# fudan-zvg/PARTNER

Measured on AMD Instinct MI355X. Metric: frames/sec polar voxelize+PFN+BEV+head, 30k-pt sweep (whole job), higher is better.
Workload: dtype f32

## Files before the change

partner_amd/csrc/pillar_rows.hip:

```cpp
#include "pn_common.h"
#include "wino_planes.h"
#include <algorithm>

namespace {

using f32x4 = __attribute__((ext_vector_type(4))) float;

#ifndef PN_ROWS_EXP
#define PN_ROWS_EXP 0
#endif
constexpr int RW_LD = 132;
constexpr int RW_MAXLIST = 256;

struct RowsArgs {
  const float* canvas;
  const uint32_t* keys;
  const int32_t* row_start;
  const float* w;
  const float* scale;
  const float* shift;
  float* planes;
  float* out;
  int B, T, R, OH, OW, Wq, in_ps, in_co, act, cout, cout_pad, out_ps, out_co, v_cap;
  unsigned plane_floats, canvas_bytes, w_bytes;
};

template <int NS>
__global__ __launch_bounds__(512) void pillar_rows_kernel(RowsArgs a) {
  extern __shared__ __attribute__((aligned(16))) float smem[];
  float* tile = smem;
  int* lists = reinterpret_cast<int*>(smem + (size_t)a.OW * RW_LD);
  int* cnt = lists + 3 * 2 * RW_MAXLIST;
  const int tid = threadIdx.x, lane = tid & 63, wv = __builtin_amdgcn_readfirstlane(tid >> 6);
  const int go = blockIdx.x;
  const int b = go / a.OH, oy = go - b * a.OH;

  int run_lo = 0, run_hi = 0;
  if (wv < 3) {
    const int iy = 2 * oy - 1 + wv;
    if (iy >= 0 && iy < a.T) {
      run_lo = a.row_start[b * a.T + iy];
      run_hi = a.row_start[b * a.T + iy + 1];
    }
  }
  {
    const f32x4 z = {0.f, 0.f, 0.f, 0.f};
    f32x4* t4 = reinterpret_cast<f32x4*>(tile);
    for (int i = tid; i < a.OW * RW_LD / 4; i += 512) t4[i] = z;
  }
  if (wv < 3) {
    const int iy = 2 * oy - 1 + wv;
    int ne = 0, no = 0;
    if (iy >= 0 && iy < a.T) {
      const int gi = b * a.T + iy;
      const int lo = min(run_lo, a.v_cap), hi = min(run_hi, a.v_cap);
      const uint32_t key0 = (uint32_t)gi * (uint32_t)a.R;
      int* le = lists + (wv * 2 + 0) * RW_MAXLIST;
      int* lo_ = lists + (wv * 2 + 1) * RW_MAXLIST;
      for (int base = lo; base < hi; base += 64) {
        const int i = base + lane;
        const bool live = i < hi;
        const int ix = live ? (int)(a.keys[i] - key0) : 0;
        const bool odd = live && (ix & 1), even = live && !(ix & 1);
        const unsigned long long me = __ballot(even), mo = __ballot(odd);
        const unsigned long long below = (1ull << lane) - 1ull;
        if (even) le[ne + __popcll(me & below)] = ix;
        if (odd) lo_[no + __popcll(mo & below)] = ix;
        ne += __popcll(me);
        no += __popcll(mo);
      }
    }
    if (lane == 0) {
      cnt[wv * 2] = ne;
      cnt[wv * 2 + 1] = no;
    }
  }
  __syncthreads();

  const __amdgpu_buffer_rsrc_t rsrc_c = __builtin_amdgcn_make_buffer_rsrc(const_cast<float*>(a.canvas), 0, a.canvas_bytes, 0x00020000);
  const __amdgpu_buffer_rsrc_t rsrc_w = __builtin_amdgcn_make_buffer_rsrc(const_cast<float*>(a.w), 0, a.w_bytes, 0x00020000);
  const int j = lane & 15, kq = lane >> 4;
  const int c0 = wv * 16;
  const bool cols_live = c0 < a.cout;
  const unsigned w_lane = (unsigned)(((c0 + j) * 4 + kq) * 16);
  const unsigned w_slab = (unsigned)a.cout_pad * 64u;
  auto load_w = [&](int tap, f32x4 (&f)[NS]) __attribute__((always_inline)) {
#pragma unroll
    for (int s = 0; s < NS; ++s)
      f[s] = __builtin_bit_cast(f32x4, __builtin_amdgcn_raw_buffer_load_b128(rsrc_w, (cols_live && !(PN_ROWS_EXP & 4)) ? w_lane : 0xffffffffu, (unsigned)(tap * NS + s) * w_slab, 0));
  };
  auto add_to_tile = [&](int ox, const f32x4 acc) __attribute__((always_inline)) {
    f32x4* p = reinterpret_cast<f32x4*>(tile + (size_t)ox * RW_LD + c0 + 4 * kq);
    *p = *p + acc;
  };
  f32x4 w0[NS], w1[NS], w2[NS];
  auto row_live = [&](int kh) { const int iy = 2 * oy - 1 + kh; return iy >= 0 && iy < a.T && !(PN_ROWS_EXP & 1); };
  if (row_live(0)) load_w(1, w1);
  else load_w(3 + 1, w1);
#pragma unroll
  for (int kh = 0; kh < 3; ++kh) {
    if (!row_live(kh)) continue;
    const int iy = 2 * oy - 1 + kh;
    const unsigned row_pix = (unsigned)(b * a.T + iy) * (unsigned)a.R;
    const int ne = cnt[kh * 2], no = cnt[kh * 2 + 1];
    const int te = (ne + 15) >> 4, nu = te + ((no + 15) >> 4);
    const int* le = lists + (kh * 2 + 0) * RW_MAXLIST;
    const int* lo_ = lists + (kh * 2 + 1) * RW_MAXLIST;
    auto unit_ix = [&](int u) {
      const bool odd = u >= te;
      const int idx = (odd ? u - te : u) * 16 + j;
      return idx < (odd ? no : ne) ? (odd ? lo_[idx] : le[idx]) : -1;
    };
    auto request = [&](int ix, f32x4 (&xf)[NS]) __attribute__((always_inline)) {
      const unsigned voff = (ix >= 0 && !(PN_ROWS_EXP & 4)) ? ((row_pix + (unsigned)ix) * (unsigned)a.in_ps + (unsigned)a.in_co + 4u * (unsigned)kq) * 4u : 0xffffffffu;
#pragma unroll
      for (int s2 = 0; s2 < NS; ++s2) xf[s2] = __builtin_bit_cast(f32x4, __builtin_amdgcn_raw_buffer_load_b128(rsrc_c, voff, (unsigned)s2 * 64u, 0));
    };
    auto unit = [&](int u, int ix, const f32x4 (&xf)[NS], int ix_next, f32x4 (&xn)[NS]) __attribute__((always_inline)) {
      if (u + 1 < nu) request(ix_next, xn);
      f32x4 p = {0.f, 0.f, 0.f, 0.f}, q = {0.f, 0.f, 0.f, 0.f};
      if (u < te) {
#pragma unroll
        for (int s2 = 0; s2 < ((PN_ROWS_EXP & 8) ? 0 : NS); s2 += 2)
#pragma unroll
          for (int m = 0; m < 4; ++m) {
            p = __builtin_amdgcn_mfma_f32_16x16x4f32(w1[s2][m], xf[s2][m], p, 0, 0, 0);
            q = __builtin_amdgcn_mfma_f32_16x16x4f32(w1[s2 + 1][m], xf[s2 + 1][m], q, 0, 0, 0);
          }
        if (ix >= 0) add_to_tile(ix >> 1, p + q);
        if (u + 1 == te && kh < 2) load_w((kh + 1) * 3 + 1, w1);
      } else {
#pragma unroll
        for (int s2 = 0; s2 < ((PN_ROWS_EXP & 8) ? 0 : NS); ++s2)
#pragma unroll
          for (int m = 0; m < 4; ++m) {
            p = __builtin_amdgcn_mfma_f32_16x16x4f32(w0[s2][m], xf[s2][m], p, 0, 0, 0);
            q = __builtin_amdgcn_mfma_f32_16x16x4f32(w2[s2][m], xf[s2][m], q, 0, 0, 0);
          }
        if (ix >= 0 && ((ix + 1) >> 1) < a.OW) add_to_tile((ix + 1) >> 1, p);
        if (ix >= 0) add_to_tile((ix - 1) >> 1, q);
      }
    };
    f32x4 xa[NS], xb[NS];
    int ixa = nu > 0 ? unit_ix(0) : -1, ixb = -1;
    if (nu > 0) request(ixa, xa);
    if (no > 0) {
      load_w(kh * 3 + 0, w0);
      load_w(kh * 3 + 2, w2);
    }
    if (te == 0 && kh < 2) load_w((kh + 1) * 3 + 1, w1);
#pragma unroll 1
    for (int u = 0; u < nu; u += 2) {
      ixb = u + 1 < nu ? unit_ix(u + 1) : -1;
      unit(u, ixa, xa, ixb, xb);
      if (u + 1 < nu) {
        ixa = u + 2 < nu ? unit_ix(u + 2) : -1;
        unit(u + 1, ixb, xb, ixa, xa);
      }
    }
  }
  __syncthreads();

  const f32x4 z = {0.f, 0.f, 0.f, 0.f};
  const int c4n = a.cout >> 2;
  if (PN_ROWS_EXP & 2) return;
  if (a.planes) {
    for (int it = tid; it < c4n * a.Wq; it += 512) {
      const int c4 = it / a.Wq, xq = it - c4 * a.Wq;
      f32x4 sc = {1.f, 1.f, 1.f, 1.f}, sh = z;
      if (a.scale) sc = *reinterpret_cast<const f32x4*>(a.scale + c4 * 4);
      if (a.shift) sh = *reinterpret_cast<const f32x4*>(a.shift + c4 * 4);
      f32x4 d[6];
#pragma unroll
      for (int i = 0; i < 6; ++i) {
        const int ox = 4 * xq - 1 + i;
        if (ox < 0 || ox >= a.OW) {
          d[i] = z;
        } else {
          const f32x4 s = *reinterpret_cast<const f32x4*>(tile + (size_t)ox * RW_LD + c4 * 4);
#pragma unroll
          for (int c = 0; c < 4; ++c) d[i][c] = pn::apply_act(fmaf(s[c], sc[c], sh[c]), a.act);
        }
      }
      f32x4 vv[6];
      pn::wino4_input_transform4(d, vv);
      pn::wino4_store_planes(a.planes, vv, c4, c4n, a.plane_floats, b, oy, xq, a.OH, a.Wq);
    }
  }
  if (a.out) {
    float* orow = a.out + ((size_t)go * a.OW) * a.out_ps + a.out_co;
    for (int it = tid; it < a.OW * c4n; it += 512) {
      const int ox = it / c4n, c4 = it - ox * c4n;
      f32x4 sc = {1.f, 1.f, 1.f, 1.f}, sh = z;
      if (a.scale) sc = *reinterpret_cast<const f32x4*>(a.scale + c4 * 4);
      if (a.shift) sh = *reinterpret_cast<const f32x4*>(a.shift + c4 * 4);
      const f32x4 s = *reinterpret_cast<const f32x4*>(tile + (size_t)ox * RW_LD + c4 * 4);
      f32x4 y;
#pragma unroll
      for (int c = 0; c < 4; ++c) y[c] = pn::apply_act(fmaf(s[c], sc[c], sh[c]), a.act);
      *reinterpret_cast<f32x4*>(orow + (size_t)ox * a.out_ps + c4 * 4) = y;
    }
  }
}

__global__ void pack_pillar_rows_weight_kernel(const float* __restrict__ w, int cout, int cin, int cout_pad, float* __restrict__ packed, size_t total) {
  for (size_t i = blockIdx.x * (size_t)blockDim.x + threadIdx.x; i < total; i += (size_t)gridDim.x * blockDim.x) {
    const int m = (int)(i & 3), kq = (int)((i >> 2) & 3);
    size_t r = i >> 4;
    const int co = (int)(r % cout_pad);
    r /= cout_pad;
    const int ns = cin / 16;
    const int s = (int)(r % ns), tap = (int)(r / ns);
    const int ci = 16 * s + 4 * kq + m;
    packed[i] = co < cout ? w[((size_t)co * cin + ci) * 9 + tap] : 0.f;
  }
}

static int rows_cout_pad(int cout) { return pn::cdiv(cout, 16) * 16; }

}

extern "C" {

int pn_pillar_conv_rows_supported(int batch, int h, int w, int cin, int cout, int stride) {
  if (stride != 2 || batch < 1 || h < 2 || w < 8 || (w & 7) || w > 2 * RW_MAXLIST) return 0;
  const int ow = (w - 1) / 2 + 1, wq = ow / 4;
  if (ow % 4 || !(wq == 16 || wq == 32 || wq == 64)) return 0;
  if (!(cin == 32 || cin == 64 || cin == 128) || cout < 4 || cout > 128 || (cout & 3)) return 0;
  return 1;
}

size_t pn_pillar_conv_rows_packed_weight_floats(int cout, int cin) { return (size_t)9 * cin * rows_cout_pad(cout); }

int pn_pack_pillar_conv_rows_weight_f32(const float* w_oihw, int cout, int cin, float* packed, pn_stream_t stream) {
  PN_REQUIRE(w_oihw && packed && cout >= 1 && cin >= 16 && cin % 16 == 0, "pack_pillar_conv_rows_weight: bad arguments");
  const size_t total = pn_pillar_conv_rows_packed_weight_floats(cout, cin);
  hipLaunchKernelGGL(pack_pillar_rows_weight_kernel, dim3((unsigned)std::min<size_t>(2048, (total + 255) / 256)), dim3(256), 0, pn::S(stream), w_oihw, cout, cin,
                     rows_cout_pad(cout), packed, total);
  return pn::check_launch("pack_pillar_rows_weight_kernel");
}

int pn_pillar_conv3x3_rows_f32(const float* canvas, int batch, int h, int w, int cin, int in_pixel_stride, int in_channel_offset, const uint32_t* unq_keys,
                               const int32_t* row_start, int v_capacity, const float* packed_rows_w, int cout, const float* scale, const float* shift, int act,
                               float* planes, float* out, int out_pixel_stride, int out_channel_offset, pn_stream_t stream) {
  PN_REQUIRE(canvas && unq_keys && row_start && packed_rows_w && (planes || out), "pillar_conv_rows: null pointer");
  PN_REQUIRE(pn_pillar_conv_rows_supported(batch, h, w, cin, cout, 2), "pillar_conv_rows: shape not covered (see pn_pillar_conv_rows_supported)");
  PN_REQUIRE(in_pixel_stride % 4 == 0 && in_channel_offset % 4 == 0 && in_channel_offset + cin <= in_pixel_stride && ((uintptr_t)canvas & 15) == 0,
             "pillar_conv_rows: the canvas slice must be 16-byte aligned");
  PN_REQUIRE(!out || (out_pixel_stride % 4 == 0 && out_channel_offset % 4 == 0 && out_channel_offset + cout <= out_pixel_stride && ((uintptr_t)out & 15) == 0),
             "pillar_conv_rows: the output slice must be 16-byte aligned");
  PN_REQUIRE(((uintptr_t)scale & 15) == 0 && ((uintptr_t)shift & 15) == 0 && ((uintptr_t)planes & 15) == 0, "pillar_conv_rows: 16-byte aligned tables");
  const unsigned long long cb = (unsigned long long)batch * h * w * in_pixel_stride * 4ull;
  PN_REQUIRE(cb < (1ull << 32), "pillar_conv_rows: canvases of 4 GiB or more are not addressable by the buffer descriptor");
  RowsArgs a{};
  a.canvas = canvas; a.keys = unq_keys; a.row_start = row_start; a.w = packed_rows_w; a.scale = scale; a.shift = shift; a.planes = planes; a.out = out;
  a.B = batch; a.T = h; a.R = w; a.OH = (h - 1) / 2 + 1; a.OW = (w - 1) / 2 + 1; a.Wq = a.OW / 4;
  a.in_ps = in_pixel_stride; a.in_co = in_channel_offset; a.act = act; a.cout = cout; a.cout_pad = rows_cout_pad(cout);
  a.out_ps = out_pixel_stride; a.out_co = out_channel_offset; a.v_cap = v_capacity;
  a.plane_floats = (unsigned)((size_t)batch * (a.OH + 2) * a.Wq * 4);
  a.canvas_bytes = (unsigned)cb;
  a.w_bytes = (unsigned)(pn_pillar_conv_rows_packed_weight_floats(cout, cin) * 4);
  const size_t smem = ((size_t)a.OW * RW_LD + 3 * 2 * RW_MAXLIST + 8) * sizeof(float);
  pn::ProfileSlot slot;
  const bool prof = pn::take_profile_slot(slot);
  hipStream_t st = pn::S(stream);
  const dim3 grid((unsigned)(batch * a.OH));
#define PN_ROWS_LAUNCH(NS)                                                                                                                  \
  do {                                                                                                                                      \
    static bool done[64] = {false};                                                                                                         \
    if (pn::first_use_on_device(done))                                                                                                      \
      (void)hipFuncSetAttribute(reinterpret_cast<const void*>(&pillar_rows_kernel<NS>), hipFuncAttributeMaxDynamicSharedMemorySize, 160 * 1024); \
    if (prof) hipExtLaunchKernelGGL(pillar_rows_kernel<NS>, grid, dim3(512), smem, st, slot.start, slot.stop, 0, a);                         \
    else hipLaunchKernelGGL(pillar_rows_kernel<NS>, grid, dim3(512), smem, st, a);                                                          \
  } while (0)
  if (cin == 128) PN_ROWS_LAUNCH(8);
  else if (cin == 64) PN_ROWS_LAUNCH(4);
  else PN_ROWS_LAUNCH(2);
#undef PN_ROWS_LAUNCH
  return pn::check_launch("pillar_rows_kernel");
}

}
```

Measured before the change: 1834.

## Split pillar-row conv blocks by output-channel band and column segment

Restructures the sparse pillar-row convolution kernel so each block handles one output-channel band (NW waves of 16 channels) and optionally a column segment with a halo, in place of a 512-thread block covering all channels of a row. This gives a larger grid with smaller LDS footprints, adds an XCD-aware block-index swizzle, and replaces the two-buffer unit ping-pong with separate even/odd loops that issue next-unit canvas loads interleaved between MFMA groups under sched_barriers. The aim is more occupancy and better latency hiding, at the cost of each block re-scanning the row's key lists and re-loading weights for its band. An env var can force the geometry, and the default picks 4-wave channel bands when OW is at least 128.

Result: no change. 1847 (median of 6 runs) (+0.7%).

```diff
diff --git a/partner_amd/csrc/pillar_rows.hip b/partner_amd/csrc/pillar_rows.hip
--- a/partner_amd/csrc/pillar_rows.hip
+++ b/partner_amd/csrc/pillar_rows.hip
@@ -1,6 +1,7 @@
 #include "pn_common.h"
 #include "wino_planes.h"
 #include <algorithm>
+#include <cstdlib>
 
 namespace {
 
@@ -9,8 +10,15 @@
 #ifndef PN_ROWS_EXP
 #define PN_ROWS_EXP 0
 #endif
-constexpr int RW_LD = 132;
 constexpr int RW_MAXLIST = 256;
+
+template <int CS, int NW>
+struct RowsGeom {
+  static constexpr int HALO = CS > 1 ? 1 : 0;
+  static constexpr int LD = 16 * NW + 4;
+  static constexpr int LCAP = RW_MAXLIST / CS + 2 * HALO;
+  static size_t smem_bytes(int ow) { return ((size_t)(ow / CS + 2 * HALO) * LD + 3 * 2 * LCAP + 8) * sizeof(float); }
+};
 
 struct RowsArgs {
   const float* canvas;
@@ -21,19 +29,28 @@
   const float* shift;
   float* planes;
   float* out;
-  int B, T, R, OH, OW, Wq, in_ps, in_co, act, cout, cout_pad, out_ps, out_co, v_cap;
+  int B, T, R, OH, OW, Wq, in_ps, in_co, act, cout, cout_pad, out_ps, out_co, v_cap, ncb;
   unsigned plane_floats, canvas_bytes, w_bytes;
 };
 
-template <int NS>
-__global__ __launch_bounds__(512) void pillar_rows_kernel(RowsArgs a) {
+template <int NS, int CS, int NW>
+__global__ __launch_bounds__(64 * NW) __attribute__((amdgpu_waves_per_eu(NW == 4 ? 3 : 2))) void pillar_rows_kernel(RowsArgs a) {
+  using G = RowsGeom<CS, NW>;
+  constexpr int HALO = G::HALO, LD = G::LD, LCAP = G::LCAP, NT = 64 * NW;
   extern __shared__ __attribute__((aligned(16))) float smem[];
+  const int OWS = a.OW / CS, TP = OWS + 2 * HALO;
   float* tile = smem;
-  int* lists = reinterpret_cast<int*>(smem + (size_t)a.OW * RW_LD);
-  int* cnt = lists + 3 * 2 * RW_MAXLIST;
+  int* lists = reinterpret_cast<int*>(smem + (size_t)TP * LD);
+  int* cnt = lists + 3 * 2 * LCAP;
   const int tid = threadIdx.x, lane = tid & 63, wv = __builtin_amdgcn_readfirstlane(tid >> 6);
-  const int go = blockIdx.x;
+  int bid = blockIdx.x;
+  if (!(PN_ROWS_EXP & 16) && !(gridDim.x & 7)) bid = (bid & 7) * (int)(gridDim.x >> 3) + (bid >> 3);
+  const int go = bid / (CS * a.ncb), band = bid - go * (CS * a.ncb);
+  const int seg = band / a.ncb, cb = band - seg * a.ncb;
   const int b = go / a.OH, oy = go - b * a.OH;
+  const int x0 = seg * OWS, x1 = x0 + OWS;
+  const int tx0 = max(x0 - HALO, 0), tx1 = min(x1 + HALO, a.OW);
+  const int ix_lo = CS > 1 ? 2 * x0 - 3 : 0, ix_hi = CS > 1 ? 2 * x1 + 1 : a.R;
 
   int run_lo = 0, run_hi = 0;
   if (wv < 3) {
@@ -46,7 +63,7 @@
   {
     const f32x4 z = {0.f, 0.f, 0.f, 0.f};
     f32x4* t4 = reinterpret_cast<f32x4*>(tile);
-    for (int i = tid; i < a.OW * RW_LD / 4; i += 512) t4[i] = z;
+    for (int i = tid; i < TP * LD / 4; i += NT) t4[i] = z;
   }
   if (wv < 3) {
     const int iy = 2 * oy - 1 + wv;
@@ -55,24 +72,26 @@
       const int gi = b * a.T + iy;
       const int lo = min(run_lo, a.v_cap), hi = min(run_hi, a.v_cap);
       const uint32_t key0 = (uint32_t)gi * (uint32_t)a.R;
-      int* le = lists + (wv * 2 + 0) * RW_MAXLIST;
-      int* lo_ = lists + (wv * 2 + 1) * RW_MAXLIST;
+      int* le = lists + (wv * 2 + 0) * LCAP;
+      int* lo_ = lists + (wv * 2 + 1) * LCAP;
       for (int base = lo; base < hi; base += 64) {
         const int i = base + lane;
-        const bool live = i < hi;
+        bool live = i < hi;
         const int ix = live ? (int)(a.keys[i] - key0) : 0;
+        live = live && ix >= ix_lo && ix <= ix_hi;
         const bool odd = live && (ix & 1), even = live && !(ix & 1);
         const unsigned long long me = __ballot(even), mo = __ballot(odd);
         const unsigned long long below = (1ull << lane) - 1ull;
-        if (even) le[ne + __popcll(me & below)] = ix;
-        if (odd) lo_[no + __popcll(mo & below)] = ix;
+        const int pe = ne + __popcll(me & below), po = no + __popcll(mo & below);
+        if (even && pe < LCAP) le[pe] = ix;
+        if (odd && po < LCAP) lo_[po] = ix;
         ne += __popcll(me);
         no += __popcll(mo);
       }
     }
     if (lane == 0) {
-      cnt[wv * 2] = ne;
-      cnt[wv * 2 + 1] = no;
+      cnt[wv * 2] = min(ne, LCAP);
+      cnt[wv * 2 + 1] = min(no, LCAP);
     }
   }
   __syncthreads();
@@ -80,7 +99,7 @@
   const __amdgpu_buffer_rsrc_t rsrc_c = __builtin_amdgcn_make_buffer_rsrc(const_cast<float*>(a.canvas), 0, a.canvas_bytes, 0x00020000);
   const __amdgpu_buffer_rsrc_t rsrc_w = __builtin_amdgcn_make_buffer_rsrc(const_cast<float*>(a.w), 0, a.w_bytes, 0x00020000);
   const int j = lane & 15, kq = lane >> 4;
-  const int c0 = wv * 16;
+  const int cl = wv * 16, c0 = cb * 16 * NW + cl;
   const bool cols_live = c0 < a.cout;
   const unsigned w_lane = (unsigned)(((c0 + j) * 4 + kq) * 16);
   const unsigned w_slab = (unsigned)a.cout_pad * 64u;
@@ -90,7 +109,8 @@
       f[s] = __builtin_bit_cast(f32x4, __builtin_amdgcn_raw_buffer_load_b128(rsrc_w, (cols_live && !(PN_ROWS_EXP & 4)) ? w_lane : 0xffffffffu, (unsigned)(tap * NS + s) * w_slab, 0));
   };
   auto add_to_tile = [&](int ox, const f32x4 acc) __attribute__((always_inline)) {
-    f32x4* p = reinterpret_cast<f32x4*>(tile + (size_t)ox * RW_LD + c0 + 4 * kq);
+    if (ox < tx0 || ox >= tx1) return;
+    f32x4* p = reinterpret_cast<f32x4*>(tile + (size_t)(ox - x0 + HALO) * LD + cl + 4 * kq);
     *p = *p + acc;
   };
   f32x4 w0[NS], w1[NS], w2[NS];
@@ -104,69 +124,88 @@
     const unsigned row_pix = (unsigned)(b * a.T + iy) * (unsigned)a.R;
     const int ne = cnt[kh * 2], no = cnt[kh * 2 + 1];
     const int te = (ne + 15) >> 4, nu = te + ((no + 15) >> 4);
-    const int* le = lists + (kh * 2 + 0) * RW_MAXLIST;
-    const int* lo_ = lists + (kh * 2 + 1) * RW_MAXLIST;
+    const int* le = lists + (kh * 2 + 0) * LCAP;
+    const int* lo_ = lists + (kh * 2 + 1) * LCAP;
     auto unit_ix = [&](int u) {
+      if (u >= nu) return -1;
       const bool odd = u >= te;
       const int idx = (odd ? u - te : u) * 16 + j;
       return idx < (odd ? no : ne) ? (odd ? lo_[idx] : le[idx]) : -1;
     };
-    auto request = [&](int ix, f32x4 (&xf)[NS]) __attribute__((always_inline)) {
-      const unsigned voff = (ix >= 0 && !(PN_ROWS_EXP & 4)) ? ((row_pix + (unsigned)ix) * (unsigned)a.in_ps + (unsigned)a.in_co + 4u * (unsigned)kq) * 4u : 0xffffffffu;
-#pragma unroll
-      for (int s2 = 0; s2 < NS; ++s2) xf[s2] = __builtin_bit_cast(f32x4, __builtin_amdgcn_raw_buffer_load_b128(rsrc_c, voff, (unsigned)s2 * 64u, 0));
+    auto canvas_off = [&](int ix) {
+      return (ix >= 0 && !(PN_ROWS_EXP & 4)) ? ((row_pix + (unsigned)ix) * (unsigned)a.in_ps + (unsigned)a.in_co + 4u * (unsigned)kq) * 4u : 0xffffffffu;
     };
-    auto unit = [&](int u, int ix, const f32x4 (&xf)[NS], int ix_next, f32x4 (&xn)[NS]) __attribute__((always_inline)) {
-      if (u + 1 < nu) request(ix_next, xn);
+    auto request = [&](unsigned voff, int s2) __attribute__((always_inline)) {
+      return __builtin_bit_cast(f32x4, __builtin_amdgcn_raw_buffer_load_b128(rsrc_c, voff, (unsigned)s2 * 64u, 0));
+    };
+    f32x4 xf[NS];
+    int ix = unit_ix(0);
+    {
+      const unsigned voff = canvas_off(ix);
+#pragma unroll
+      for (int s2 = 0; s2 < NS; ++s2) xf[s2] = request(voff, s2);
+    }
+    if (no > 0) {
+      load_w(kh * 3 + 0, w0);
+      load_w(kh * 3 + 2, w2);
+    }
+#pragma unroll 1
+    for (int u = 0; u < te; ++u) {
+      const int ix_next = unit_ix(u + 1);
+      const unsigned voff = canvas_off(ix_next);
       f32x4 p = {0.f, 0.f, 0.f, 0.f}, q = {0.f, 0.f, 0.f, 0.f};
-      if (u < te) {
-#pragma unroll
-        for (int s2 = 0; s2 < ((PN_ROWS_EXP & 8) ? 0 : NS); s2 += 2)
+#pragma unroll
+      for (int s2 = 0; s2 < NS; s2 += 2) {
+        if (!(PN_ROWS_EXP & 8)) {
 #pragma unroll
           for (int m = 0; m < 4; ++m) {
             p = __builtin_amdgcn_mfma_f32_16x16x4f32(w1[s2][m], xf[s2][m], p, 0, 0, 0);
             q = __builtin_amdgcn_mfma_f32_16x16x4f32(w1[s2 + 1][m], xf[s2 + 1][m], q, 0, 0, 0);
           }
-        if (ix >= 0) add_to_tile(ix >> 1, p + q);
-        if (u + 1 == te && kh < 2) load_w((kh + 1) * 3 + 1, w1);
-      } else {
-#pragma unroll
-        for (int s2 = 0; s2 < ((PN_ROWS_EXP & 8) ? 0 : NS); ++s2)
+        }
+        __builtin_amdgcn_sched_barrier(0);
+        xf[s2] = request(voff, s2);
+        xf[s2 + 1] = request(voff, s2 + 1);
+        __builtin_amdgcn_sched_barrier(0);
+      }
+      if (ix >= 0) add_to_tile(ix >> 1, p + q);
+      ix = ix_next;
+    }
+    if (kh < 2) load_w((kh + 1) * 3 + 1, w1);
+#pragma unroll 1
+    for (int u = te; u < nu; ++u) {
+      const int ix_next = unit_ix(u + 1);
+      const unsigned voff = canvas_off(ix_next);
+      f32x4 p = {0.f, 0.f, 0.f, 0.f}, q = {0.f, 0.f, 0.f, 0.f};
+#pragma unroll
+      for (int s2 = 0; s2 < NS; ++s2) {
+        if (!(PN_ROWS_EXP & 8)) {
 #pragma unroll
           for (int m = 0; m < 4; ++m) {
             p = __builtin_amdgcn_mfma_f32_16x16x4f32(w0[s2][m], xf[s2][m], p, 0, 0, 0);
             q = __builtin_amdgcn_mfma_f32_16x16x4f32(w2[s2][m], xf[s2][m], q, 0, 0, 0);
           }
-        if (ix >= 0 && ((ix + 1) >> 1) < a.OW) add_to_tile((ix + 1) >> 1, p);
-        if (ix >= 0) add_to_tile((ix - 1) >> 1, q);
-      }
-    };
-    f32x4 xa[NS], xb[NS];
-    int ixa = nu > 0 ? unit_ix(0) : -1, ixb = -1;
-    if (nu > 0) request(ixa, xa);
-    if (no > 0) {
-      load_w(kh * 3 + 0, w0);
-      load_w(kh * 3 + 2, w2);
-    }
-    if (te == 0 && kh < 2) load_w((kh + 1) * 3 + 1, w1);
-#pragma unroll 1
-    for (int u = 0; u < nu; u += 2) {
-      ixb = u + 1 < nu ? unit_ix(u + 1) : -1;
-      unit(u, ixa, xa, ixb, xb);
-      if (u + 1 < nu) {
-        ixa = u + 2 < nu ? unit_ix(u + 2) : -1;
-        unit(u + 1, ixb, xb, ixa, xa);
-      }
+        }
+        __builtin_amdgcn_sched_barrier(0);
+        xf[s2] = request(voff, s2);
+        __builtin_amdgcn_sched_barrier(0);
+      }
+      if (ix >= 0) {
+        add_to_tile((ix + 1) >> 1, p);
+        add_to_tile((ix - 1) >> 1, q);
+      }
+      ix = ix_next;
     }
   }
   __syncthreads();
 
   const f32x4 z = {0.f, 0.f, 0.f, 0.f};
-  const int c4n = a.cout >> 2;
+  const int c4n = a.cout >> 2, c4b = cb * 4 * NW, nq = min(c4n - c4b, 4 * NW);
   if (PN_ROWS_EXP & 2) return;
   if (a.planes) {
-    for (int it = tid; it < c4n * a.Wq; it += 512) {
-      const int c4 = it / a.Wq, xq = it - c4 * a.Wq;
+    const int WqS = OWS >> 2;
+    for (int it = tid; it < nq * WqS; it += NT) {
+      const int c4l = it / WqS, xq = (x0 >> 2) + it - c4l * WqS, c4 = c4b + c4l;
       f32x4 sc = {1.f, 1.f, 1.f, 1.f}, sh = z;
       if (a.scale) sc = *reinterpret_cast<const f32x4*>(a.scale + c4 * 4);
       if (a.shift) sh = *reinterpret_cast<const f32x4*>(a.shift + c4 * 4);
@@ -177,7 +216,7 @@
         if (ox < 0 || ox >= a.OW) {
           d[i] = z;
         } else {
-          const f32x4 s = *reinterpret_cast<const f32x4*>(tile + (size_t)ox * RW_LD + c4 * 4);
+          const f32x4 s = *reinterpret_cast<const f32x4*>(tile + (size_t)(ox - x0 + HALO) * LD + c4l * 4);
 #pragma unroll
           for (int c = 0; c < 4; ++c) d[i][c] = pn::apply_act(fmaf(s[c], sc[c], sh[c]), a.act);
         }
@@ -188,17 +227,17 @@
     }
   }
   if (a.out) {
-    float* orow = a.out + ((size_t)go * a.OW) * a.out_ps + a.out_co;
-    for (int it = tid; it < a.OW * c4n; it += 512) {
-      const int ox = it / c4n, c4 = it - ox * c4n;
+    float* orow = a.out + ((size_t)go * a.OW + x0) * a.out_ps + a.out_co + c4b * 4;
+    for (int it = tid; it < OWS * nq; it += NT) {
+      const int oxl = it / nq, c4l = it - oxl * nq, c4 = c4b + c4l;
       f32x4 sc = {1.f, 1.f, 1.f, 1.f}, sh = z;
       if (a.scale) sc = *reinterpret_cast<const f32x4*>(a.scale + c4 * 4);
       if (a.shift) sh = *reinterpret_cast<const f32x4*>(a.shift + c4 * 4);
-      const f32x4 s = *reinterpret_cast<const f32x4*>(tile + (size_t)ox * RW_LD + c4 * 4);
+      const f32x4 s = *reinterpret_cast<const f32x4*>(tile + (size_t)(oxl + HALO) * LD + c4l * 4);
       f32x4 y;
 #pragma unroll
       for (int c = 0; c < 4; ++c) y[c] = pn::apply_act(fmaf(s[c], sc[c], sh[c]), a.act);
-      *reinterpret_cast<f32x4*>(orow + (size_t)ox * a.out_ps + c4 * 4) = y;
+      *reinterpret_cast<f32x4*>(orow + (size_t)oxl * a.out_ps + c4l * 4) = y;
     }
   }
 }
@@ -217,6 +256,36 @@
 }
 
 static int rows_cout_pad(int cout) { return pn::cdiv(cout, 16) * 16; }
+
+static int rows_geometry(int ow, int cout, int cin) {
+  static const int force = [] { const char* e = getenv("PN_PILLAR_ROWS_BLOCK"); return e ? atoi(e) : -1; }();
+  (void)cout, (void)cin;
+  int g = ow >= 128 ? 2 : 0;
+  if (force >= 0 && force <= 3) g = force;
+  if (ow / 4 == 16 && (g & 1)) g = g == 1 ? 2 : 0;
+  return g;
+}
+
+template <int NS, int CS, int NW>
+static void launch_rows(RowsArgs& a, hipStream_t st, bool prof, const pn::ProfileSlot& slot) {
+  const size_t smem = RowsGeom<CS, NW>::smem_bytes(a.OW);
+  static bool done[64] = {false};
+  if (pn::first_use_on_device(done))
+    (void)hipFuncSetAttribute(reinterpret_cast<const void*>(&pillar_rows_kernel<NS, CS, NW>), hipFuncAttributeMaxDynamicSharedMemorySize,
+                              (int)RowsGeom<CS, NW>::smem_bytes(RW_MAXLIST));
+  a.ncb = pn::cdiv(a.cout, 16 * NW);
+  const dim3 grid((unsigned)(a.B * a.OH * CS * a.ncb));
+  if (prof) hipExtLaunchKernelGGL((pillar_rows_kernel<NS, CS, NW>), grid, dim3(64 * NW), smem, st, slot.start, slot.stop, 0, a);
+  else hipLaunchKernelGGL((pillar_rows_kernel<NS, CS, NW>), grid, dim3(64 * NW), smem, st, a);
+}
+
+template <int NS>
+static void launch_rows_geometry(int g, RowsArgs& a, hipStream_t st, bool prof, const pn::ProfileSlot& slot) {
+  if (g == 1) launch_rows<NS, 2, 4>(a, st, prof, slot);
+  else if (g == 2) launch_rows<NS, 1, 4>(a, st, prof, slot);
+  else if (g == 3) launch_rows<NS, 2, 8>(a, st, prof, slot);
+  else launch_rows<NS, 1, 8>(a, st, prof, slot);
+}
 
 }
 
@@ -260,23 +329,13 @@
   a.plane_floats = (unsigned)((size_t)batch * (a.OH + 2) * a.Wq * 4);
   a.canvas_bytes = (unsigned)cb;
   a.w_bytes = (unsigned)(pn_pillar_conv_rows_packed_weight_floats(cout, cin) * 4);
-  const size_t smem = ((size_t)a.OW * RW_LD + 3 * 2 * RW_MAXLIST + 8) * sizeof(float);
   pn::ProfileSlot slot;
   const bool prof = pn::take_profile_slot(slot);
   hipStream_t st = pn::S(stream);
-  const dim3 grid((unsigned)(batch * a.OH));
-#define PN_ROWS_LAUNCH(NS)                                                                                                                  \
-  do {                                                                                                                                      \
-    static bool done[64] = {false};                                                                                                         \
-    if (pn::first_use_on_device(done))                                                                                                      \
-      (void)hipFuncSetAttribute(reinterpret_cast<const void*>(&pillar_rows_kernel<NS>), hipFuncAttributeMaxDynamicSharedMemorySize, 160 * 1024); \
-    if (prof) hipExtLaunchKernelGGL(pillar_rows_kernel<NS>, grid, dim3(512), smem, st, slot.start, slot.stop, 0, a);                         \
-    else hipLaunchKernelGGL(pillar_rows_kernel<NS>, grid, dim3(512), smem, st, a);                                                          \
-  } while (0)
-  if (cin == 128) PN_ROWS_LAUNCH(8);
-  else if (cin == 64) PN_ROWS_LAUNCH(4);
-  else PN_ROWS_LAUNCH(2);
-#undef PN_ROWS_LAUNCH
+  const int g = rows_geometry(a.OW, cout, cin);
+  if (cin == 128) launch_rows_geometry<8>(g, a, st, prof, slot);
+  else if (cin == 64) launch_rows_geometry<4>(g, a, st, prof, slot);
+  else launch_rows_geometry<2>(g, a, st, prof, slot);
   return pn::check_launch("pillar_rows_kernel");
 }
 
```
